# sair-lab/localization

Hardware: AMD Instinct MI355X
Metric: localization updates/sec (8-anchor UWB, batch=65k) (higher is better)
Workload: dtype f64

## Files before the change

### include/localization_amd.h

```cpp
#ifndef LOCALIZATION_AMD_H
#define LOCALIZATION_AMD_H

#include <stddef.h>
#include <stdint.h>

#ifdef __cplusplus
extern "C" {
#endif

#define LOC_ABI_VERSION 4

typedef enum loc_status {
    LOC_OK = 0,
    LOC_ERR_INVALID = -1,
    LOC_ERR_NO_DEVICE = -2,
    LOC_ERR_HIP = -3,
    LOC_ERR_UNKNOWN_NODE = -4,
    LOC_ERR_UNSUPPORTED = -5,
    LOC_ERR_SINGULAR = -6
} loc_status;

enum { LOC_JAC_ANALYTIC = 0, LOC_JAC_NUMERIC_G2O = 1 };

const char* loc_last_error(void);
// ... 33 lines not shown

int loc_snapshot_set_positions(loc_snapshot* s, const double* pos_soa_host);
int loc_snapshot_get_positions(loc_snapshot* s, double* pos_soa_host);
void* loc_snapshot_positions_device(loc_snapshot* s);
int64_t loc_snapshot_epochs_done(const loc_snapshot* s);
int loc_snapshot_set_epochs_done(loc_snapshot* s, int64_t epochs);

int loc_snapshot_pack_ranges_host(const loc_snapshot* s, int32_t epochs, const float* src_kmb, float* dst_tiles,
                                  float pad_value);

int loc_snapshot_solve_device(loc_snapshot* s, int32_t epochs, const float* dist_dev, const float* err_dev,
                              double* out_pos_dev, double* out_chi2_dev, uint8_t* out_trials_dev,
                              void* hip_stream);

int loc_snapshot_solve_host(loc_snapshot* s, int32_t epochs, const float* dist_tiles_host,
                            const float* err_tiles_host, double* out_pos_host, double* out_chi2_host,
                            uint8_t* out_trials_host);

int loc_snapshot_solve_host_kmb(loc_snapshot* s, int32_t epochs, const float* dist_kmb_host, const float* err_kmb_host,
                                double* out_pos_host, double* out_chi2_host, uint8_t* out_trials_host);

int loc_snapshot_solve_device_cov(loc_snapshot* s, int32_t epochs, const float* dist_dev, const float* err_dev,
                                  double* out_pos_dev, double* out_chi2_dev, uint8_t* out_trials_dev,
                                  double* out_cov_dev, int32_t* out_cov_mask_dev, int32_t* out_cov_status_dev, void* hip_stream);
int loc_snapshot_solve_host_kmb_cov(loc_snapshot* s, int32_t epochs, const float* dist_kmb_host, const float* err_kmb_host,
                                    double* out_pos_host, double* out_chi2_host, uint8_t* out_trials_host,
                                    double* out_cov_host, int32_t* out_cov_mask_host, int32_t* out_cov_status_host);

int loc_host_alloc(void** out, size_t bytes);
int loc_host_free(void* p);

int loc_snapshot_timing_begin(loc_snapshot* s, int32_t max_launches);
int loc_snapshot_timing_end(loc_snapshot* s, int32_t* n_launches, double* total_ms, double* avg_ms);


typedef struct loc_window loc_window;
typedef struct loc_window_caps {
    int32_t nv_max, nr_max, np_max, ns_max;
    int32_t bw_max;
} loc_window_caps;

int loc_window_create(loc_window** out, int32_t device, int64_t batch, const loc_window_caps* caps,
                      int32_t n_anchors, const double* anchors_xyz_host, int32_t maximum_iteration);
int loc_window_destroy(loc_window* w);
int loc_window_set_anchors(loc_window* w, int32_t n_anchors, const double* anchors_xyz_host);
size_t loc_window_lds_bytes(const loc_window_caps* caps);
int loc_window_solve_host(loc_window* w, int64_t n_instances, const int32_t* counts, double* poses,
                          const int32_t* r_idx, const double* r_val, const int32_t* p_idx, const double* p_val,
                          const int32_t* s_idx, const double* s_val, double* result);
int loc_window_last_kernel_ms(loc_window* w, double* ms);
int loc_window_set_endpoint1_offsets(loc_window* w, int64_t n_instances, const double* off1_xyz);
int loc_window_set_prior_information(loc_window* w, int64_t n_instances, const double* pinfo);
int loc_window_set_jacobian(loc_window* w, int32_t jacobian);
int loc_window_set_ordering(loc_window* w, int32_t natural);
int loc_window_set_chain_threshold(loc_window* w, int64_t min_batch);
enum { LOC_WINDOW_KERNEL_NONE = -1, LOC_WINDOW_KERNEL_GENERAL = 0, LOC_WINDOW_KERNEL_CHAIN = 1, LOC_WINDOW_KERNEL_CHAIN3 = 2, LOC_WINDOW_KERNEL_ARROW3 = 3, LOC_WINDOW_KERNEL_TREE = 4,
       LOC_WINDOW_KERNEL_TREE_LANE = 5 ,
       LOC_WINDOW_KERNEL_WAVE3 = 6 ,
       LOC_WINDOW_KERNEL_WAVE6 = 7 ,
       LOC_WINDOW_KERNEL_WAVE6S = 8  };
int loc_window_last_kernel_kind(const loc_window* w, int32_t* kind);
int loc_window_set_option(loc_window* w, const char* name, int64_t value);
int loc_window_last_host_timing(const loc_window* w, double* validate_topology_run_cached);
int loc_window_upload(loc_window* w, int64_t n_instances, const int32_t* counts, const double* poses,
                      const int32_t* r_idx, const double* r_val, const int32_t* p_idx, const double* p_val,
                      const int32_t* s_idx, const double* s_val);
// ... 193 lines not shown
```

### localization_amd/_lib.py

```python
import ctypes as C
import os

_HERE = os.path.dirname(os.path.abspath(__file__))
_SO = os.environ.get("LOCALIZATION_AMD_LIB") or os.path.join(_HERE, "liblocalization_amd.so")
_LIB = None

LOC_OK = 0
LOC_ERR_NO_DEVICE = -2
JAC_ANALYTIC = 0
JAC_NUMERIC_G2O = 1


class LocalizationAmdError(RuntimeError):
    def __init__(self, code, msg):
        super().__init__(f"localization_amd error {code}: {msg}")
        self.code = code


class SnapshotParams(C.Structure):
    _fields_ = [("maximum_iteration", C.c_int32), ("distance_outlier", C.c_double), ("gate_warmup_epochs", C.c_int32), ("jacobian", C.c_int32),
                ("lanes_per_instance", C.c_int32), ("block_threads", C.c_int32)]


class FusionParams(C.Structure):
    _fields_ = [("maximum_iteration", C.c_int32), ("distance_outlier", C.c_double), ("gate_warmup_epochs", C.c_int32),
                ("antenna_offset", C.c_double * 3), ("block_threads", C.c_int32), ("jacobian", C.c_int32)]


def library_path():
    return _SO


EXPORTED_SYMBOLS = [
    "loc_last_error", "loc_abi_version", "loc_device_count", "loc_shard_bounds", "loc_shard_plan",
    "loc_snapshot_default_params", "loc_snapshot_create", "loc_snapshot_destroy", "loc_snapshot_batch",
    "loc_snapshot_anchor_groups", "loc_snapshot_lanes_per_instance", "loc_snapshot_range_floats",
    "loc_snapshot_set_positions", "loc_snapshot_get_positions", "loc_snapshot_positions_device",
    "loc_snapshot_epochs_done", "loc_snapshot_set_epochs_done",
    "loc_snapshot_pack_ranges_host", "loc_snapshot_solve_device", "loc_snapshot_solve_host",
    "loc_snapshot_solve_host_kmb", "loc_snapshot_solve_device_cov", "loc_snapshot_solve_host_kmb_cov", "loc_host_alloc", "loc_host_free",
    "loc_snapshot_timing_begin", "loc_snapshot_timing_end",
    "loc_window_create", "loc_window_destroy", "loc_window_set_anchors", "loc_window_lds_bytes", "loc_window_solve_host",
    "loc_window_last_kernel_ms", "loc_window_set_endpoint1_offsets", "loc_window_set_prior_information", "loc_window_set_jacobian", "loc_window_set_ordering", "loc_window_set_chain_threshold", "loc_window_last_kernel_kind", "loc_window_set_option", "loc_window_last_host_timing", "loc_window_upload", "loc_window_upload_dev",
    "loc_window_solve_resident", "loc_window_download", "loc_window_poses_device", "loc_window_result_device",
    "loc_window_timing_begin", "loc_window_timing_end",
    "loc_window_covariance_host", "loc_window_covariance_resident", "loc_window_last_covariance_ms", "loc_window_covariance_plan",
    "loc_window_marginal_prior_host", "loc_window_joint_covariance_host", "loc_window_joint_covariance_resident", "loc_window_joint_covariance_plan",
    "loc_window_slide_resident", "loc_window_slide_resident_dev", "loc_window_slide_plain_resident_dev", "loc_window_download_tables",
    "loc_window_edge_chi2_host", "loc_window_edge_chi2_resident", "loc_window_prune_resident",
    "loc_window_publish_resident", "loc_window_path_resident",
    "loc_window_set_message_config", "loc_window_message_rows_dev", "loc_window_push_messages_resident_dev",
    "loc_node_default_config", "loc_node_create", "loc_node_destroy", "loc_node_add_range", "loc_node_add_imu",
    "loc_node_add_pose", "loc_node_add_twist", "loc_node_add_lidar", "loc_node_add_rl_range", "loc_node_solve", "loc_node_get_path",
    "loc_node_number_measurements", "loc_node_last_timing", "loc_node_last_kernel_kind", "loc_node_flush_tail", "loc_node_set_deferred", "loc_node_solve_pending", "loc_nodes_solve_batch",
    "loc_nodes_release_batch_cache",
    "loc_fusion_default_params", "loc_fusion_create", "loc_fusion_destroy", "loc_fusion_set_poses", "loc_fusion_get_poses",
    "loc_fusion_solve_device", "loc_fusion_solve_host", "loc_fusion_solve_host_kmb", "loc_fusion_last_kernel_ms", "loc_fusion_timing_begin", "loc_fusion_timing_end",
    "loc_fusion_solve_device_cov", "loc_fusion_solve_host_kmb_cov",
]


def lib():
    global _LIB
    if _LIB is not None:
        return _LIB
    if not os.path.exists(_SO):
        raise LocalizationAmdError(-100, f"{_SO} is missing: build it with `python -c 'import __graft_entry__ as g; "
                                   "g.build()'` (hipcc --offload-arch=gfx950). There is no CPU fallback.")
    L = C.CDLL(_SO)
    vp, dp, fp = C.c_void_p, C.POINTER(C.c_double), C.POINTER(C.c_float)
    L.loc_last_error.restype = C.c_char_p
    L.loc_abi_version.restype = C.c_int32
    L.loc_device_count.restype = C.c_int32
    L.loc_shard_bounds.argtypes = [C.c_int64, C.c_int32, C.c_int32, C.POINTER(C.c_int64), C.POINTER(C.c_int64)]
    L.loc_shard_plan.argtypes = [C.c_int64, C.c_int32, C.c_int32, C.c_void_p]
    L.loc_snapshot_default_params.argtypes = [C.POINTER(SnapshotParams)]
    L.loc_snapshot_default_params.restype = None
    L.loc_snapshot_create.argtypes = [C.POINTER(vp), C.c_int32, C.c_int64, C.c_int32, dp, C.POINTER(SnapshotParams)]
    L.loc_snapshot_destroy.argtypes = [vp]
    L.loc_snapshot_batch.argtypes = [vp]; L.loc_snapshot_batch.restype = C.c_int64
    L.loc_snapshot_anchor_groups.argtypes = [vp]; L.loc_snapshot_anchor_groups.restype = C.c_int32
    L.loc_snapshot_lanes_per_instance.argtypes = [vp]; L.loc_snapshot_lanes_per_instance.restype = C.c_int32
    L.loc_snapshot_range_floats.argtypes = [vp, C.c_int32]; L.loc_snapshot_range_floats.restype = C.c_size_t
    L.loc_snapshot_set_positions.argtypes = [vp, dp]
    L.loc_snapshot_get_positions.argtypes = [vp, dp]
    L.loc_snapshot_positions_device.argtypes = [vp]; L.loc_snapshot_positions_device.restype = vp
    L.loc_snapshot_epochs_done.argtypes = [vp]; L.loc_snapshot_epochs_done.restype = C.c_int64
    L.loc_snapshot_set_epochs_done.argtypes = [vp, C.c_int64]
    L.loc_snapshot_pack_ranges_host.argtypes = [vp, C.c_int32, fp, fp, C.c_float]
    L.loc_snapshot_solve_device.argtypes = [vp, C.c_int32, vp, vp, vp, vp, vp, vp]
    L.loc_snapshot_solve_host.argtypes = [vp, C.c_int32, fp, fp, dp, dp, C.POINTER(C.c_uint8)]
    L.loc_snapshot_solve_host_kmb.argtypes = [vp, C.c_int32, vp, vp, vp, vp, vp]
    L.loc_snapshot_solve_device_cov.argtypes = [vp, C.c_int32] + [vp] * 9
    L.loc_snapshot_solve_host_kmb_cov.argtypes = [vp, C.c_int32] + [vp] * 8
    L.loc_host_alloc.argtypes = [C.POINTER(vp), C.c_size_t]
    L.loc_host_free.argtypes = [vp]
    L.loc_snapshot_timing_begin.argtypes = [vp, C.c_int32]
    L.loc_snapshot_timing_end.argtypes = [vp, C.POINTER(C.c_int32), dp, dp]
    ip = C.POINTER(C.c_int32)
    L.loc_window_create.argtypes = [C.POINTER(vp), C.c_int32, C.c_int64, vp, C.c_int32, dp, C.c_int32]
    L.loc_window_destroy.argtypes = [vp]
    L.loc_window_set_anchors.argtypes = [vp, C.c_int32, dp]
    L.loc_window_lds_bytes.argtypes = [vp]; L.loc_window_lds_bytes.restype = C.c_size_t
    L.loc_window_solve_host.argtypes = [vp, C.c_int64, ip, dp, ip, dp, ip, dp, ip, dp, dp]
    L.loc_window_last_kernel_ms.argtypes = [vp, dp]
    L.loc_window_set_jacobian.argtypes = [vp, C.c_int32]
    L.loc_window_set_endpoint1_offsets.argtypes = [vp, C.c_int64, dp]
    L.loc_window_set_prior_information.argtypes = [vp, C.c_int64, dp]
    L.loc_window_set_ordering.argtypes = [vp, C.c_int32]
    L.loc_window_set_chain_threshold.argtypes = [vp, C.c_int64]
    L.loc_window_last_kernel_kind.argtypes = [vp, ip]
    L.loc_window_upload.argtypes = [vp, C.c_int64, ip, dp, ip, dp, ip, dp, ip, dp]
    L.loc_window_upload_dev.argtypes = [vp, vp, C.c_int64] + [vp] * 9
    L.loc_window_solve_resident.argtypes = [vp, vp]
    L.loc_window_download.argtypes = [vp, dp, dp]
    L.loc_window_poses_device.argtypes = [vp]; L.loc_window_poses_device.restype = vp
    L.loc_window_result_device.argtypes = [vp]; L.loc_window_result_device.restype = vp
    L.loc_window_timing_begin.argtypes = [vp, C.c_int32]
    L.loc_window_timing_end.argtypes = [vp, ip, dp, dp]
    L.loc_window_covariance_host.argtypes = [vp, C.c_int64, ip, dp, ip, dp, ip, dp, ip, dp, dp, ip, ip]
    L.loc_window_marginal_prior_host.argtypes = [vp, C.c_int64, ip, dp, ip, dp, ip, dp, ip, dp, ip, ip, dp, dp, dp, ip, ip]
    L.loc_window_covariance_resident.argtypes = [vp, vp, vp, vp, vp]
    L.loc_window_last_covariance_ms.argtypes = [vp, dp]
    L.loc_window_covariance_plan.argtypes = [vp, C.c_int64, ip, ip, ip, C.POINTER(C.c_int64), C.POINTER(C.c_size_t)]
    L.loc_window_joint_covariance_host.argtypes = [vp, C.c_int64, ip, dp, ip, dp, ip, dp, ip, dp, C.c_int32, ip, ip, dp, ip, ip, dp]
    L.loc_window_joint_covariance_resident.argtypes = [vp, vp, C.c_int32, ip, ip, vp, vp, vp, vp]
    L.loc_window_joint_covariance_plan.argtypes = [vp, C.c_int64, ip, ip, ip, C.c_int32, ip, ip, C.POINTER(C.c_int64), C.POINTER(C.c_size_t)]
    L.loc_window_set_option.argtypes = [vp, C.c_char_p, C.c_int64]
    L.loc_window_slide_resident.argtypes = [vp, vp, ip, dp, C.c_int32, ip, ip, dp, C.c_int32, ip, dp, vp, vp, vp, vp]
    L.loc_window_slide_resident_dev.argtypes = [vp, vp, vp, vp, C.c_int32, vp, vp, vp, C.c_int32, vp, vp, vp, vp, vp, vp, vp]
    L.loc_window_slide_plain_resident_dev.argtypes = [vp, vp, vp, vp, C.c_int32, vp, vp, vp, C.c_int32, vp, vp, C.c_int32, vp, vp, vp, vp, vp]
# ... 134 lines not shown
```

### localization_amd/csrc/capi.cpp

```cpp
#include <algorithm>
#include <cmath>
#include <cstdio>
#include <cstring>
#include <new>
#include <string>
#include <vector>

#include "capi_host.h"
#include "snapshot_kernel.h"

static thread_local std::string g_last_error;

int locamd_fail(int code, const char* what) {
    g_last_error = what ? what : "";
    return code;
}
int locamd_fail_hip(hipError_t e, const char* where) {
    g_last_error = std::string(where) + ": " + hipGetErrorString(e);
    return LOC_ERR_HIP;
}

struct loc_snapshot {
    int device = 0;
    long long B = 0;
    int M = 0, M4 = 0, M_PAD = 0;
    int lpi = 1;
    loc_snapshot_params prm{};
    double* d_anchors = nullptr;
    double* d_pos = nullptr;
    hipStream_t own_stream = nullptr;
    float *d_dist = nullptr, *d_err = nullptr;
    double *d_out_pos = nullptr, *d_out_chi2 = nullptr;
    uint8_t* d_out_trials = nullptr;
    size_t staged_epochs = 0;
    long long epochs_done = 0;
    locamd::HostPipeline pipe;
    locamd::LaunchTimer timer;
};

extern "C" {

const char* loc_last_error(void) { return g_last_error.c_str(); }
int32_t loc_abi_version(void) { return LOC_ABI_VERSION; }

int32_t loc_device_count(void) {
    int n = 0;
    if (hipGetDeviceCount(&n) != hipSuccess) return 0;
    return n;
}

int loc_shard_bounds(int64_t total, int32_t rank, int32_t world, int64_t* lo, int64_t* hi) {
    if (total < 0 || world <= 0 || rank < 0 || rank >= world || !lo || !hi) return locamd_fail(LOC_ERR_INVALID, "loc_shard_bounds arguments");
    const int64_t per = (total + world - 1) / world;
    const int64_t a = rank * per < total ? rank * per : total;
    *lo = a;
    *hi = a + per < total ? a + per : total;
    return LOC_OK;
}

int loc_shard_plan(int64_t total, int32_t world, int32_t devices_per_node, loc_shard* out) {
    if (total < 0 || world <= 0 || !out) return locamd_fail(LOC_ERR_INVALID, "loc_shard_plan arguments");
    if (devices_per_node <= 0) {
        devices_per_node = loc_device_count();
        if (devices_per_node <= 0) return locamd_fail(LOC_ERR_NO_DEVICE, "no HIP device visible: pass devices_per_node explicitly");
    }
    for (int32_t r = 0; r < world; ++r) {
        out[r].rank = r; out[r].world = world; out[r].device = r % devices_per_node; out[r].reserved = 0;
        const int rc = loc_shard_bounds(total, r, world, &out[r].lo, &out[r].hi);
// ... 105 lines not shown
    if (!s || !src || !dst || epochs <= 0) return locamd_fail(LOC_ERR_INVALID, "pack_ranges");
    const size_t B = (size_t)s->B;
    for (int k = 0; k < epochs; ++k)
        for (int g = 0; g < s->M4; ++g)
            for (int j = 0; j < 4; ++j) {
                const int m = 4 * g + j;
                float* d = dst + (((size_t)k * s->M4 + g) * B) * 4 + j;
                if (m < s->M) {
                    const float* sp = src + ((size_t)k * s->M + m) * B;
                    for (size_t b = 0; b < B; ++b) d[4 * b] = sp[b];
                } else {
                    for (size_t b = 0; b < B; ++b) d[4 * b] = pad_value;
                }
            }
    return LOC_OK;
}

}

static int solve_device(loc_snapshot* s, int32_t epochs, const float* dist_dev, const float* err_dev, double* out_pos_dev,
                        double* out_chi2_dev, uint8_t* out_trials_dev, double* cov, int32_t* cov_mask, int32_t* cov_status, void* hip_stream) {
    if (epochs <= 0 || !dist_dev || !err_dev || !out_pos_dev || !out_chi2_dev) return locamd_fail(LOC_ERR_INVALID, "solve arguments");
    if (((uintptr_t)dist_dev | (uintptr_t)err_dev) & 15u) return locamd_fail(LOC_ERR_INVALID, "range tiles must be 16-byte aligned");
    LOC_HIP(hipSetDevice(s->device));
    hipStream_t st = hip_stream ? (hipStream_t)hip_stream : s->own_stream;
    locamd::SnapshotArgs a;
    a.dist = dist_dev; a.err = err_dev; a.pos = s->d_pos; a.out_pos = out_pos_dev; a.out_chi2 = out_chi2_dev;
    a.out_trials = out_trials_dev; a.anchors = s->d_anchors; a.B = s->B; a.K = epochs; a.M4 = s->M4;
    a.iterations = s->prm.maximum_iteration; a.gate = s->prm.distance_outlier;
    {
        long long left = (long long)s->prm.gate_warmup_epochs - s->epochs_done;
        a.gate_from_epoch = left > 0 ? (int)(left > epochs ? epochs : left) : 0;
    }
    LOC_HIP(s->timer.start(st));
    hipError_t e;
    if (!cov) {
        e = locamd::launch_snapshot(a, s->M_PAD, s->lpi, s->prm.jacobian, s->prm.block_threads, st);
    } else {
        locamd::SnapshotCovArgs ca;
        static_cast<locamd::SnapshotArgs&>(ca) = a;
        ca.out_cov = cov; ca.out_cov_mask = cov_mask; ca.out_cov_status = cov_status;
        e = locamd::launch_snapshot_cov(ca, s->M_PAD, s->lpi, s->prm.jacobian, s->prm.block_threads, st);
    }
    if (e != hipSuccess) return locamd_fail_hip(e, "launch_snapshot");
    LOC_HIP(s->timer.stop(st));
    s->epochs_done += epochs;
    return LOC_OK;
}

extern "C" {

int loc_snapshot_solve_device(loc_snapshot* s, int32_t epochs, const float* dist_dev, const float* err_dev,
                              double* out_pos_dev, double* out_chi2_dev, uint8_t* out_trials_dev, void* hip_stream) {
    if (!s) return locamd_fail(LOC_ERR_INVALID, "null handle");
    return solve_device(s, epochs, dist_dev, err_dev, out_pos_dev, out_chi2_dev, out_trials_dev, nullptr, nullptr, nullptr, hip_stream);
}

int loc_snapshot_solve_device_cov(loc_snapshot* s, int32_t epochs, const float* dist_dev, const float* err_dev,
                                  double* out_pos_dev, double* out_chi2_dev, uint8_t* out_trials_dev,
                                  double* out_cov_dev, int32_t* out_cov_mask_dev, int32_t* out_cov_status_dev, void* hip_stream) {
    if (!s) return locamd_fail(LOC_ERR_INVALID, "null handle");
    if (!out_cov_dev || !out_cov_mask_dev || !out_cov_status_dev) return locamd_fail(LOC_ERR_INVALID, "covariance outputs: all three are required");
    return solve_device(s, epochs, dist_dev, err_dev, out_pos_dev, out_chi2_dev, out_trials_dev, out_cov_dev, out_cov_mask_dev,
                        out_cov_status_dev, hip_stream);
}

// ... 38 lines not shown
                     return solve_device(s, kc, s->d_dist + toff, s->d_err + toff, s->d_out_pos + 3 * o, s->d_out_chi2 + o, s->d_out_trials + o,
                                         cov_h ? p.d_cov + 6 * o : nullptr, cov_h ? p.d_cov_mask + o : nullptr, cov_h ? p.d_cov_status + o : nullptr, s->own_stream);
                 });
}

extern "C" {

int loc_snapshot_solve_host_kmb(loc_snapshot* s, int32_t epochs, const float* dist_kmb, const float* err_kmb,
                                double* out_pos_h, double* out_chi2_h, uint8_t* out_trials_h) {
    if (!s) return locamd_fail(LOC_ERR_INVALID, "null handle");
    return solve_host_kmb(s, epochs, dist_kmb, err_kmb, out_pos_h, out_chi2_h, out_trials_h, nullptr, nullptr, nullptr);
}

int loc_snapshot_solve_host_kmb_cov(loc_snapshot* s, int32_t epochs, const float* dist_kmb, const float* err_kmb,
                                    double* out_pos_h, double* out_chi2_h, uint8_t* out_trials_h,
                                    double* out_cov_h, int32_t* out_cov_mask_h, int32_t* out_cov_status_h) {
    if (!s) return locamd_fail(LOC_ERR_INVALID, "null handle");
    if (!out_cov_h || !out_cov_mask_h || !out_cov_status_h) return locamd_fail(LOC_ERR_INVALID, "covariance outputs: all three are required");
    return solve_host_kmb(s, epochs, dist_kmb, err_kmb, out_pos_h, out_chi2_h, out_trials_h, out_cov_h, out_cov_mask_h, out_cov_status_h);
}

int loc_host_alloc(void** out, size_t bytes) {
    if (!out || bytes == 0) return locamd_fail(LOC_ERR_INVALID, "loc_host_alloc");
    *out = nullptr;
    LOC_HIP(hipHostMalloc(out, bytes, hipHostMallocDefault));
    return LOC_OK;
}
int loc_host_free(void* p) {
    if (!p) return LOC_OK;
    LOC_HIP(hipHostFree(p));
    return LOC_OK;
}

int loc_snapshot_timing_begin(loc_snapshot* s, int32_t max_launches) {
    return s ? s->timer.begin(s->device, max_launches) : locamd_fail(LOC_ERR_INVALID, "timing_begin");
}
int loc_snapshot_timing_end(loc_snapshot* s, int32_t* n_launches, double* total_ms, double* avg_ms) {
    return s ? s->timer.end(s->device, n_launches, total_ms, avg_ms) : locamd_fail(LOC_ERR_INVALID, "timing_end");
}

}
```

### localization_amd/csrc/lm_damping.h

```cpp
#pragma once
#include <hip/hip_runtime.h>
#include <math.h>

namespace locamd {
namespace {

constexpr double lm_tau = 1e-5;
constexpr double lm_good_lo = 1.0 / 3.0;
constexpr double lm_good_hi = 2.0 / 3.0;
constexpr int lm_max_trials = 10;
constexpr double lm_scale_eps = 1e-3;

__device__ __forceinline__ double lm_lambda_accepted(double lambda, double rho) {
    const double r21 = 2.0 * rho - 1.0;
    double alpha = 1.0 - r21 * r21 * r21;
    alpha = fmin(alpha, lm_good_hi);
    return lambda * fmax(lm_good_lo, alpha);
}

}
}
```

### localization_amd/csrc/snapshot_kernel.h

```cpp
#pragma once
#include <hip/hip_runtime.h>
#include <stdint.h>

namespace locamd {

struct SnapshotArgs {
    const float* dist;
    const float* err;
    double* pos;
    double* out_pos;
    double* out_chi2;
    uint8_t* out_trials;
    const double* anchors;
    long long B;
    int K;
    int M4;
    int iterations;
    double gate;
    int gate_from_epoch;
};

struct SnapshotCovArgs : SnapshotArgs {
    double* out_cov;
    int32_t* out_cov_mask;
    int32_t* out_cov_status;
};

hipError_t launch_snapshot(const SnapshotArgs& a, int m_pad, int lpi, int jac, int block_threads, hipStream_t stream);
hipError_t launch_snapshot_cov(const SnapshotCovArgs& a, int m_pad, int lpi, int jac, int block_threads, hipStream_t stream);
bool snapshot_supported(int m_pad, int lpi);
hipError_t launch_pack_kmb(const float* src_kmb, float* dst_tiles, long long B, int M, int M4, int K, float pad, hipStream_t stream);

}
```

### localization_amd/csrc/snapshot_kernel.hip

```cpp
#include "snapshot_kernel.h"
#include "device_math.h"
#include "lm_damping.h"
#include "cov_device.h"

#include <float.h>
#include <math.h>

#include <type_traits>

namespace locamd {

namespace {

template <int CTRL>
__device__ __forceinline__ double dpp_move(double v) {
    int lo = __double2loint(v), hi = __double2hiint(v);
    lo = __builtin_amdgcn_update_dpp(0, lo, CTRL, 0xF, 0xF, false);
    hi = __builtin_amdgcn_update_dpp(0, hi, CTRL, 0xF, 0xF, false);
    return __hiloint2double(hi, lo);
}
constexpr int DPP_QUAD_XOR1 = 0xB1;
constexpr int DPP_QUAD_XOR2 = 0x4E;
constexpr int DPP_ROW_HALF_MIRROR = 0x141;

template <int LPI>
__device__ __forceinline__ double group_sum(double v) {
    if constexpr (LPI >= 2) v += dpp_move<DPP_QUAD_XOR1>(v);
    if constexpr (LPI >= 4) v += dpp_move<DPP_QUAD_XOR2>(v);
    if constexpr (LPI >= 8) v += dpp_move<DPP_ROW_HALF_MIRROR>(v);
    return v;
}
template <int LPI>
__device__ __forceinline__ double group_prod(double v) {
    if constexpr (LPI >= 2) v *= dpp_move<DPP_QUAD_XOR1>(v);
    if constexpr (LPI >= 4) v *= dpp_move<DPP_QUAD_XOR2>(v);
    if constexpr (LPI >= 8) v *= dpp_move<DPP_ROW_HALF_MIRROR>(v);
    return v;
}

struct System {
    double h00, h01, h02, h11, h12, h22;
    double b0, b1, b2;
    double rchi;
    double chi;
};

#pragma clang fp contract(off)
__device__ __forceinline__ double range_norm_plain(double dx, double dy, double dz) {
    return sqrt_ieee_unscaled(dx * dx + dy * dy + dz * dz);
}
__device__ __forceinline__ double range_sq_plain(double dx, double dy, double dz) { return dx * dx + dy * dy + dz * dz; }
#pragma clang fp contract(fast)

template <int LPI, int APL, int JAC>
__device__ __forceinline__ System evaluate(const double px, const double py, const double pz,
                                           const double (&ax)[APL], const double (&ay)[APL], const double (&az)[APL],
                                           const double (&d)[APL], double (&w)[APL], const double gate) {
    System s = {0, 0, 0, 0, 0, 0, 0, 0, 0, 0, 0};
    double prod = 1.0;
    int kexp = 0;
#pragma unroll
    for (int j = 0; j < APL; ++j) {
        const double dx = px - ax[j], dy = py - ay[j], dz = pz - az[j];
        double n, jx, jy, jz;
        if constexpr (JAC == 0) {
            const double n2 = fmax(dx * dx + dy * dy + dz * dz, 1e-300);
            double inv;
            sqrt_and_rsqrt_fast(n2, n, inv);
            jx = -dx * inv; jy = -dy * inv; jz = -dz * inv;
        } else {
// ... 72 lines not shown
    if constexpr (APL % 4 == 0) {
#pragma unroll
        for (int q4 = 0; q4 < APL / 4; ++q4) {
            const long long idx = (k * a.M4 + (m0 / 4 + q4)) * B + inst;
            const float4 dv = reinterpret_cast<const float4*>(a.dist)[idx];
            const float4 sv = reinterpret_cast<const float4*>(a.err)[idx];
            df[4 * q4 + 0] = dv.x; df[4 * q4 + 1] = dv.y; df[4 * q4 + 2] = dv.z; df[4 * q4 + 3] = dv.w;
            sf[4 * q4 + 0] = sv.x; sf[4 * q4 + 1] = sv.y; sf[4 * q4 + 2] = sv.z; sf[4 * q4 + 3] = sv.w;
        }
    } else if constexpr (APL == 2) {
        const long long idx = ((k * a.M4 + m0 / 4) * B + inst) * 2 + (m0 % 4) / 2;
        const float2 dv = reinterpret_cast<const float2*>(a.dist)[idx];
        const float2 sv = reinterpret_cast<const float2*>(a.err)[idx];
        df[0] = dv.x; df[1] = dv.y; sf[0] = sv.x; sf[1] = sv.y;
    } else {
        static_assert(APL == 1 || APL == 2 || APL % 4 == 0, "anchors per lane");
        const long long idx = ((k * a.M4 + m0 / 4) * B + inst) * 4 + (m0 % 4);
        df[0] = a.dist[idx]; sf[0] = a.err[idx];
    }
}
template <int APL>
__device__ __forceinline__ void ingest(const float (&df)[APL], const float (&sf)[APL], double (&d)[APL], double (&w)[APL]) {
#pragma unroll
    for (int j = 0; j < APL; ++j) {
        const double dd = (double)df[j], ss = (double)sf[j];
        const bool valid = (ss > 0.0) && (ss < DBL_MAX) && (fabs(dd) < DBL_MAX);
        const double cov = valid ? ss * ss : 1.0;
        const double mask = valid ? 1.0 : 0.0;
        d[j] = valid ? dd : 0.0;
        w[j] = fast_rcp(cov) * mask;
    }
}

template <int APL> struct SnapshotLds {
    static constexpr int NEXT_BYTES = APL * 256 * 16;
    static constexpr int RAW_BYTES = (APL % 4 == 0) ? (2 * (APL / 4) * 256 * 16) : 0;
    static constexpr int BYTES = NEXT_BYTES + RAW_BYTES;
};

typedef __attribute__((address_space(3))) void* lds_void_ptr;
typedef const __attribute__((address_space(1))) void* glb_void_ptr;

template <int LPI, int APL, int JAC, bool COV>
__global__ void __launch_bounds__(256) snapshot_lm_kernel(const std::conditional_t<COV, SnapshotCovArgs, SnapshotArgs> a) {
    __shared__ __attribute__((aligned(16))) char lds_bytes[SnapshotLds<APL>::BYTES];
    double2* const s_next = reinterpret_cast<double2*>(lds_bytes);
    float4* const s_raw = reinterpret_cast<float4*>(lds_bytes + SnapshotLds<APL>::NEXT_BYTES);
    const int tib = threadIdx.x;
    const long long tid = (long long)blockIdx.x * blockDim.x + tib;
    const long long inst = tid / LPI;
    const int g = (int)(tid % LPI);
    const long long B = a.B;
    const int K = a.K;
    const bool live = (inst < B) && K > 0;
    const long long ld_inst = live ? inst : 0;
    bool exhausted = !live;

    double ax[APL], ay[APL], az[APL];
    const int m0 = g * APL;
#pragma unroll
    for (int j = 0; j < APL; ++j) {
        ax[j] = a.anchors[(m0 + j) * 3 + 0];
        ay[j] = a.anchors[(m0 + j) * 3 + 1];
        az[j] = a.anchors[(m0 + j) * 3 + 2];
    }

    auto put_next = [&](const double (&dd)[APL], const double (&ww)[APL]) {
#pragma unroll
        for (int j = 0; j < APL; ++j) s_next[j * 256 + tib] = make_double2(dd[j], ww[j]);
    };
    auto take_next = [&](double (&dd)[APL], double (&ww)[APL]) {
        typedef double v2f64 __attribute__((ext_vector_type(2)));
        const unsigned addr = (unsigned)(unsigned long long)(s_next + tib);
        v2f64 v[APL];
#pragma unroll
        for (int j = 0; j < APL; ++j) asm volatile("ds_read_b128 %0, %1 offset:%2" : "=v"(v[j]) : "v"(addr), "n"(j * 4096));
        if constexpr (APL == 8) {
            asm volatile("s_waitcnt lgkmcnt(0)" : "+v"(v[0]), "+v"(v[1]), "+v"(v[2]), "+v"(v[3]), "+v"(v[4]), "+v"(v[5]), "+v"(v[6]), "+v"(v[7]) :: "memory");
        } else {
#pragma unroll
// ... 28 lines not shown
            }
        } else {
            load_epoch<APL>(a, ke, m0, ld_inst, df, sf);
        }
        ingest<APL>(df, sf, dd, ww);
    };

    double px = 0, py = 0, pz = 0;
    double d[APL], w[APL];
    if (live) { px = a.pos[0 * B + inst]; py = a.pos[1 * B + inst]; pz = a.pos[2 * B + inst]; }
    {
        float df0[APL], sf0[APL];
        load_epoch<APL>(a, 0, m0, ld_inst, df0, sf0);
        ingest<APL>(df0, sf0, d, w);
        if (K > 1) {
            double dn[APL], wn[APL];
            load_epoch<APL>(a, 1, m0, ld_inst, df0, sf0);
            ingest<APL>(df0, sf0, dn, wn);
            put_next(dn, wn);
        }
        if (K > 2) prefetch(2);
    }
    asm volatile("" : "+v"(px), "+v"(py), "+v"(pz));

    System cur = {1, 0, 0, 1, 0, 1, 0, 0, 0, 0, 0};
    double cur_chi = 0, last_chi = 0, lambda = 1.0, ni = 2.0;
    int c = 0;
    int k = 0;
    int it = 0, q = 0, trials = 0;
    bool init = true;
    bool waiting = false;

    while (__any(!exhausted)) {
        const bool active = !exhausted && !waiting;
        double x0, x1, x2;
        const bool ok2 = solve3(cur, lambda, x0, x1, x2) && !init;
        if (!ok2) { x0 = 0.0; x1 = 0.0; x2 = 0.0; }
        const double tx = px + x0, ty = py + x1, tz = pz + x2;
        const bool gate_now = active && init && (a.gate > 0.0) && (k >= a.gate_from_epoch);
        const System tr = evaluate<LPI, APL, JAC>(tx, ty, tz, ax, ay, az, d, w, gate_now ? a.gate : DBL_MAX);

        const bool first = active && init;
        const bool lm = active && !init;
        const double temp_chi = ok2 ? tr.rchi : DBL_MAX;
        double scale = x0 * __builtin_fma(lambda, x0, cur.b0) + x1 * __builtin_fma(lambda, x1, cur.b1) +
                       x2 * __builtin_fma(lambda, x2, cur.b2);
        scale += lm_scale_eps;
        const double rho = (cur_chi - temp_chi) * fast_rcp(scale);
        const bool accept = lm && (rho > 0.0) && (fabs(temp_chi) < DBL_MAX) && ok2;
        if (first || accept) {
            cur = tr;
            cur_chi = tr.rchi;
            px = tx; py = ty; pz = tz;
        }
        const double lam_acc = lm_lambda_accepted(lambda, rho);
        const double lam_first = lm_tau * fmax(fabs(tr.h00), fmax(fabs(tr.h11), fabs(tr.h22)));
        lambda = first ? lam_first : (accept ? lam_acc : (lm ? lambda * ni : lambda));
        ni = (first || accept) ? 2.0 : (lm ? ni * 2.0 : ni);
        last_chi = active ? tr.chi : last_chi;
        trials = first ? 0 : trials + (lm ? 1 : 0);
        q = first ? 0 : q + (lm ? 1 : 0);
        const bool end_iter = lm && !((rho < 0.0) && (q < lm_max_trials));
        it = first ? 0 : it + (end_iter ? 1 : 0);
        const bool finished = (first && ((a.iterations <= 0) || !((tr.h00 + tr.h11 + tr.h22) > 0.0))) ||
                              (end_iter && ((q == lm_max_trials) || (rho == 0.0) || (it >= a.iterations)));
        q = end_iter ? 0 : q;
        init = active ? false : init;

        if (__any(finished)) {
            if (finished) {
                if (g == 0) {
                    a.out_pos[((long long)k * 3 + 0) * B + inst] = px;
                    a.out_pos[((long long)k * 3 + 1) * B + inst] = py;
                    a.out_pos[((long long)k * 3 + 2) * B + inst] = pz;
                    a.out_chi2[(long long)k * B + inst] = last_chi;
                    if (a.out_trials) a.out_trials[(long long)k * B + inst] = (uint8_t)(trials > 255 ? 255 : trials);
                    if constexpr (COV) {
                        double hc[6] = {cur.h00, cur.h01, cur.h02, cur.h11, cur.h12, cur.h22};
                        int msk;
                        const bool cok = cov_invert_packed<3>(hc, msk);
#pragma unroll
                        for (int i = 0; i < 6; ++i) a.out_cov[((long long)k * 6 + i) * B + inst] = hc[i];
                        a.out_cov_mask[(long long)k * B + inst] = msk;
                        a.out_cov_status[(long long)k * B + inst] = cok ? 0 : -6;
                    }
                }
                if (k + 1 >= K) {
                    exhausted = true;
                    if (g == 0) { a.pos[0 * B + inst] = px; a.pos[1 * B + inst] = py; a.pos[2 * B + inst] = pz; }
                } else if (k == c) {
                    take_next(d, w);
                    k = c + 1;
                    init = true;
                } else {
                    waiting = true;
                }
            }
        }
        if (!__any(!exhausted && k == c)) {
            ++c;
            if (c + 1 < K) {
                double dn[APL], wn[APL];
                consume(c + 1, dn, wn);
                put_next(dn, wn);
                asm volatile("" ::: "memory");
                if (c + 2 < K) prefetch(c + 2);
                if (waiting) {
#pragma unroll
                    for (int j = 0; j < APL; ++j) { d[j] = dn[j]; w[j] = wn[j]; }
                    k = c + 1;
                    init = true;
                    waiting = false;
                }
            }
        }
    }
}

template <int LPI, int APL, int JAC, bool COV, class Args>
hipError_t launch_one(const Args& a, int block_threads, hipStream_t stream) {
    const long long lanes = a.B * LPI;
    const long long blocks = (lanes + block_threads - 1) / block_threads;
    if (blocks <= 0 || blocks > 0x7fffffffLL) return hipErrorInvalidValue;
    hipLaunchKernelGGL((snapshot_lm_kernel<LPI, APL, JAC, COV>), dim3((unsigned)blocks), dim3((unsigned)block_threads), 0, stream, a);
    return hipGetLastError();
}

template <int LPI, int APL, bool COV, class Args>
hipError_t launch_jac(const Args& a, int jac, int block_threads, hipStream_t stream) {
    return jac == 0 ? launch_one<LPI, APL, 0, COV>(a, block_threads, stream) : launch_one<LPI, APL, 1, COV>(a, block_threads, stream);
}

template <bool COV, class Args>
hipError_t launch_mapping(const Args& a, int m_pad, int lpi, int jac, int block_threads, hipStream_t stream) {
    if (!snapshot_supported(m_pad, lpi)) return hipErrorInvalidValue;
    if (block_threads <= 0) block_threads = 256;
    if (block_threads % 64 || block_threads > 256) return hipErrorInvalidValue;
    switch (m_pad * 100 + lpi) {
        case 401: return launch_jac<1, 4, COV>(a, jac, block_threads, stream);
        case 402: return launch_jac<2, 2, COV>(a, jac, block_threads, stream);
        case 404: return launch_jac<4, 1, COV>(a, jac, block_threads, stream);
        case 801: return launch_jac<1, 8, COV>(a, jac, block_threads, stream);
        case 802: return launch_jac<2, 4, COV>(a, jac, block_threads, stream);
        case 804: return launch_jac<4, 2, COV>(a, jac, block_threads, stream);
        case 808: return launch_jac<8, 1, COV>(a, jac, block_threads, stream);
        case 1201: return launch_jac<1, 12, COV>(a, jac, block_threads, stream);
// ... 58 lines not shown
```

### localization_amd/snapshot.py

```python
import ctypes as C

import numpy as np

from . import _lib
from ._lib import SnapshotParams, check, lib


def pack_ranges(x_kmb, pad_value=0.0):
    x = np.ascontiguousarray(x_kmb, dtype=np.float32)
    K, M, B = x.shape
    M4 = (M + 3) // 4
    out = np.full((K, M4 * 4, B), pad_value, dtype=np.float32)
    out[:, :M, :] = x
    return np.ascontiguousarray(out.reshape(K, M4, 4, B).transpose(0, 1, 3, 2))


def unpack_ranges(tiles, M):
    t = np.asarray(tiles)
    K, M4, B, _ = t.shape
    return np.ascontiguousarray(t.transpose(0, 1, 3, 2).reshape(K, M4 * 4, B)[:, :M, :])


class SnapshotSolver(_lib.EpochSolver):
    _prefix = "loc_snapshot"

    def __init__(self, anchors, batch, maximum_iteration=10, distance_outlier=1.0, jacobian="numeric",
                 lanes_per_instance=0, block_threads=0, device=0, gate_warmup_epochs=1):
        import torch
        self.torch = torch
        L = lib()
        if L.loc_device_count() <= 0 or not torch.cuda.is_available():
            raise _lib.LocalizationAmdError(_lib.LOC_ERR_NO_DEVICE,
                                            "no HIP device visible: localization_amd has no CPU fallback")
        anchors = np.ascontiguousarray(anchors, dtype=np.float64)
        assert anchors.ndim == 2 and anchors.shape[1] == 3
        self.M = anchors.shape[0]
        self.B = int(batch)
        self.device = int(device)
        self.dev = torch.device("cuda", self.device)
        prm = SnapshotParams()
        L.loc_snapshot_default_params(C.byref(prm))
        prm.maximum_iteration = int(maximum_iteration)
        prm.distance_outlier = float(distance_outlier)
        prm.gate_warmup_epochs = int(gate_warmup_epochs)
        prm.jacobian = {"analytic": _lib.JAC_ANALYTIC, "numeric": _lib.JAC_NUMERIC_G2O,
                        "numeric_g2o": _lib.JAC_NUMERIC_G2O}[jacobian]
        prm.lanes_per_instance = int(lanes_per_instance)
        prm.block_threads = int(block_threads)
        h = C.c_void_p()
        check(L.loc_snapshot_create(C.byref(h), self.device, self.B, self.M,
                                    anchors.ctypes.data_as(C.POINTER(C.c_double)), C.byref(prm)))
        self.h = h
        self.L = L
        self.M4 = L.loc_snapshot_anchor_groups(h)
        self.lanes_per_instance = L.loc_snapshot_lanes_per_instance(h)

    def set_positions(self, pos_3b):
        p = np.ascontiguousarray(pos_3b, dtype=np.float64)
        assert p.shape == (3, self.B)
        check(self.L.loc_snapshot_set_positions(self.h, p.ctypes.data_as(C.POINTER(C.c_double))))

    def get_positions(self):
        p = np.zeros((3, self.B), dtype=np.float64)
        check(self.L.loc_snapshot_get_positions(self.h, p.ctypes.data_as(C.POINTER(C.c_double))))
        return p

    def to_device_tiles(self, x_kmb, pad_value=0.0):
        return self.torch.from_numpy(pack_ranges(x_kmb, pad_value)).to(self.dev)

    def alloc_outputs(self, K, trials=True, covariance=False):
        return self._device_outputs(K, 3, 6, trials, covariance)

    def solve_device(self, dist_tiles, err_tiles, out_pos, out_chi2, out_trials=None, out_cov=None, out_cov_mask=None, out_cov_status=None):
        t = self.torch
        K = dist_tiles.shape[0]
        assert tuple(dist_tiles.shape) == (K, self.M4, self.B, 4) and dist_tiles.dtype == t.float32
        assert tuple(err_tiles.shape) == tuple(dist_tiles.shape) and err_tiles.dtype == t.float32
        assert dist_tiles.is_contiguous() and err_tiles.is_contiguous()
        assert tuple(out_pos.shape) == (K, 3, self.B) and out_pos.dtype == t.float64 and out_pos.is_contiguous()
        assert tuple(out_chi2.shape) == (K, self.B) and out_chi2.dtype == t.float64 and out_chi2.is_contiguous()
        if out_trials is not None:
            assert tuple(out_trials.shape) == (K, self.B) and out_trials.dtype == t.uint8
        for x in (dist_tiles, err_tiles, out_pos, out_chi2):
            assert x.device == self.dev
        cov = self._cov_device_args((out_cov, out_cov_mask, out_cov_status), K, 6, self.dev)
        fn = self.L.loc_snapshot_solve_device_cov if cov else self.L.loc_snapshot_solve_device
        check(fn(self.h, K, dist_tiles.data_ptr(), err_tiles.data_ptr(), out_pos.data_ptr(), out_chi2.data_ptr(),
                 out_trials.data_ptr() if out_trials is not None else None, *cov, C.c_void_p(t.cuda.current_stream(self.dev).cuda_stream)))
# ... 27 lines not shown
```

Measured before the change: 1.996 billion.

## Let idle wavefront lanes speculatively run LM damping trials for stalled lanes

When some lanes in a wavefront are exhausted or waiting while another lane is stuck retrying rejected Levenberg-Marquardt steps, the idle lanes borrow that lane's linear system and try successive lambda values from the rejection ladder in parallel. The first helper whose trial ends the iteration has its state copied back to the owner via readlane, which shortens the serial trial chain that causes divergence in the wave. The cost is a large amount of cross-lane traffic each loop, extra LDS to save the helpers' own positions, and added register pressure. Optional per-wave counters record how often helping happens.

Result: slower. 1.900 billion (-4.8%).

```diff
diff --git a/include/localization_amd.h b/include/localization_amd.h
--- a/include/localization_amd.h
+++ b/include/localization_amd.h
@@ -89,6 +89,10 @@
 
 int loc_snapshot_timing_begin(loc_snapshot* s, int32_t max_launches);
 int loc_snapshot_timing_end(loc_snapshot* s, int32_t* n_launches, double* total_ms, double* avg_ms);
+
+int loc_snapshot_set_option(loc_snapshot* s, const char* name, int64_t value);
+int64_t loc_snapshot_counter_words(const loc_snapshot* s);
+int loc_snapshot_set_counters(loc_snapshot* s, uint32_t* counters_dev, int64_t words);
 
 
 typedef struct loc_window loc_window;
diff --git a/localization_amd/_lib.py b/localization_amd/_lib.py
--- a/localization_amd/_lib.py
+++ b/localization_amd/_lib.py
@@ -40,6 +40,7 @@
     "loc_snapshot_pack_ranges_host", "loc_snapshot_solve_device", "loc_snapshot_solve_host",
     "loc_snapshot_solve_host_kmb", "loc_snapshot_solve_device_cov", "loc_snapshot_solve_host_kmb_cov", "loc_host_alloc", "loc_host_free",
     "loc_snapshot_timing_begin", "loc_snapshot_timing_end",
+    "loc_snapshot_set_option", "loc_snapshot_counter_words", "loc_snapshot_set_counters",
     "loc_window_create", "loc_window_destroy", "loc_window_set_anchors", "loc_window_lds_bytes", "loc_window_solve_host",
     "loc_window_last_kernel_ms", "loc_window_set_endpoint1_offsets", "loc_window_set_prior_information", "loc_window_set_jacobian", "loc_window_set_ordering", "loc_window_set_chain_threshold", "loc_window_last_kernel_kind", "loc_window_set_option", "loc_window_last_host_timing", "loc_window_upload", "loc_window_upload_dev",
     "loc_window_solve_resident", "loc_window_download", "loc_window_poses_device", "loc_window_result_device",
@@ -97,6 +98,9 @@
     L.loc_host_free.argtypes = [vp]
     L.loc_snapshot_timing_begin.argtypes = [vp, C.c_int32]
     L.loc_snapshot_timing_end.argtypes = [vp, C.POINTER(C.c_int32), dp, dp]
+    L.loc_snapshot_set_option.argtypes = [vp, C.c_char_p, C.c_int64]
+    L.loc_snapshot_counter_words.argtypes = [vp]; L.loc_snapshot_counter_words.restype = C.c_int64
+    L.loc_snapshot_set_counters.argtypes = [vp, vp, C.c_int64]
     ip = C.POINTER(C.c_int32)
     L.loc_window_create.argtypes = [C.POINTER(vp), C.c_int32, C.c_int64, vp, C.c_int32, dp, C.c_int32]
     L.loc_window_destroy.argtypes = [vp]
diff --git a/localization_amd/csrc/capi.cpp b/localization_amd/csrc/capi.cpp
--- a/localization_amd/csrc/capi.cpp
+++ b/localization_amd/csrc/capi.cpp
@@ -34,6 +34,8 @@
     uint8_t* d_out_trials = nullptr;
     size_t staged_epochs = 0;
     long long epochs_done = 0;
+    int trial_helpers = 1;
+    uint32_t* d_counters = nullptr;
     locamd::HostPipeline pipe;
     locamd::LaunchTimer timer;
 };
@@ -205,6 +207,7 @@
         long long left = (long long)s->prm.gate_warmup_epochs - s->epochs_done;
         a.gate_from_epoch = left > 0 ? (int)(left > epochs ? epochs : left) : 0;
     }
+    a.trial_helpers = s->trial_helpers; a.counters = s->d_counters;
     LOC_HIP(s->timer.start(st));
     hipError_t e;
     if (!cov) {
@@ -309,6 +312,22 @@
     return LOC_OK;
 }
 
+int loc_snapshot_set_option(loc_snapshot* s, const char* name, int64_t value) {
+    if (!s || !name) return locamd_fail(LOC_ERR_INVALID, "loc_snapshot_set_option arguments");
+    if (!std::strcmp(name, "trial_helpers")) { s->trial_helpers = value != 0; return LOC_OK; }
+    return locamd_fail(LOC_ERR_INVALID, "loc_snapshot_set_option: unknown option");
+}
+int64_t loc_snapshot_counter_words(const loc_snapshot* s) {
+    return s ? locamd::kSnapshotCounterWords * locamd::snapshot_waves(s->B, s->lpi, s->prm.block_threads) : 0;
+}
+int loc_snapshot_set_counters(loc_snapshot* s, uint32_t* counters_dev, int64_t words) {
+    if (!s) return locamd_fail(LOC_ERR_INVALID, "null handle");
+    if (counters_dev && (words < loc_snapshot_counter_words(s) || ((uintptr_t)counters_dev & 3u)))
+        return locamd_fail(LOC_ERR_INVALID, "loc_snapshot_set_counters: block smaller than loc_snapshot_counter_words, or misaligned");
+    s->d_counters = counters_dev;
+    return LOC_OK;
+}
+
 int loc_snapshot_timing_begin(loc_snapshot* s, int32_t max_launches) {
     return s ? s->timer.begin(s->device, max_launches) : locamd_fail(LOC_ERR_INVALID, "timing_begin");
 }
diff --git a/localization_amd/csrc/lm_damping.h b/localization_amd/csrc/lm_damping.h
--- a/localization_amd/csrc/lm_damping.h
+++ b/localization_amd/csrc/lm_damping.h
@@ -1,6 +1,12 @@
 #pragma once
 #include <hip/hip_runtime.h>
 #include <math.h>
+
+#if defined(__HIPCC__)
+#define LOCAMD_LM_HD __host__ __device__
+#else
+#define LOCAMD_LM_HD
+#endif
 
 namespace locamd {
 namespace {
@@ -18,5 +24,29 @@
     return lambda * fmax(lm_good_lo, alpha);
 }
 
+
+LOCAMD_LM_HD inline void lm_reject_step(double& lambda, double& nu) {
+    lambda *= nu;
+    nu *= 2.0;
+}
+LOCAMD_LM_HD inline void lm_reject_ladder(double& lambda, double& nu, int steps) {
+    for (int i = 0; i < lm_max_trials - 1; ++i) {
+        double l = lambda, n = nu;
+        lm_reject_step(l, n);
+        lambda = i < steps ? l : lambda;
+        nu = i < steps ? n : nu;
+    }
+}
+LOCAMD_LM_HD inline bool lm_trial_ends(double rho, int q) { return !((rho < 0.0) && (q < lm_max_trials)); }
+LOCAMD_LM_HD inline int lm_ladder_helpers(int q, int idle) {
+    const int room = lm_max_trials - 1 - q;
+    return idle < room ? (idle < 0 ? 0 : idle) : (room < 0 ? 0 : room);
+}
+LOCAMD_LM_HD inline int lm_ladder_winner(bool own_ends, unsigned long long helper_ends, unsigned long long helpers) {
+    if (own_ends || helpers == 0) return -1;
+    helper_ends &= helpers;
+    return helper_ends ? __builtin_ctzll(helper_ends) : 63 - __builtin_clzll(helpers);
+}
+
 }
 }
diff --git a/localization_amd/csrc/snapshot_kernel.h b/localization_amd/csrc/snapshot_kernel.h
--- a/localization_amd/csrc/snapshot_kernel.h
+++ b/localization_amd/csrc/snapshot_kernel.h
@@ -18,7 +18,15 @@
     int iterations;
     double gate;
     int gate_from_epoch;
+    int trial_helpers;
+    uint32_t* counters;
 };
+constexpr int kSnapshotCounterWords = 4;
+constexpr bool snapshot_trial_helpers(int lpi, int apl) { return lpi == 1 && apl <= 8; }
+inline long long snapshot_waves(long long B, int lpi, int block_threads) {
+    const long long lanes = B * lpi, blocks = (lanes + block_threads - 1) / block_threads;
+    return blocks * (block_threads / 64);
+}
 
 struct SnapshotCovArgs : SnapshotArgs {
     double* out_cov;
diff --git a/localization_amd/csrc/snapshot_kernel.hip b/localization_amd/csrc/snapshot_kernel.hip
--- a/localization_amd/csrc/snapshot_kernel.hip
+++ b/localization_amd/csrc/snapshot_kernel.hip
@@ -36,6 +36,12 @@
     if constexpr (LPI >= 4) v *= dpp_move<DPP_QUAD_XOR2>(v);
     if constexpr (LPI >= 8) v *= dpp_move<DPP_ROW_HALF_MIRROR>(v);
     return v;
+}
+
+__device__ __forceinline__ int lane_value(int v, int lane) { return __builtin_amdgcn_readlane(v, lane); }
+__device__ __forceinline__ double lane_value(double v, int lane) {
+    const int lo = __builtin_amdgcn_readlane(__double2loint(v), lane), hi = __builtin_amdgcn_readlane(__double2hiint(v), lane);
+    return __hiloint2double(hi, lo);
 }
 
 struct System {
@@ -174,10 +180,11 @@
     }
 }
 
-template <int APL> struct SnapshotLds {
+template <int APL, int LPI> struct SnapshotLds {
     static constexpr int NEXT_BYTES = APL * 256 * 16;
     static constexpr int RAW_BYTES = (APL % 4 == 0) ? (2 * (APL / 4) * 256 * 16) : 0;
-    static constexpr int BYTES = NEXT_BYTES + RAW_BYTES;
+    static constexpr int OWN_BYTES = snapshot_trial_helpers(LPI, APL) ? 3 * 256 * 8 : 0;
+    static constexpr int BYTES = NEXT_BYTES + RAW_BYTES + OWN_BYTES;
 };
 
 typedef __attribute__((address_space(3))) void* lds_void_ptr;
@@ -185,9 +192,12 @@
 
 template <int LPI, int APL, int JAC, bool COV>
 __global__ void __launch_bounds__(256) snapshot_lm_kernel(const std::conditional_t<COV, SnapshotCovArgs, SnapshotArgs> a) {
-    __shared__ __attribute__((aligned(16))) char lds_bytes[SnapshotLds<APL>::BYTES];
+    typedef SnapshotLds<APL, LPI> Lds;
+    constexpr bool HELPERS = snapshot_trial_helpers(LPI, APL);
+    __shared__ __attribute__((aligned(16))) char lds_bytes[Lds::BYTES];
     double2* const s_next = reinterpret_cast<double2*>(lds_bytes);
-    float4* const s_raw = reinterpret_cast<float4*>(lds_bytes + SnapshotLds<APL>::NEXT_BYTES);
+    float4* const s_raw = reinterpret_cast<float4*>(lds_bytes + Lds::NEXT_BYTES);
+    [[maybe_unused]] double* const s_own = reinterpret_cast<double*>(lds_bytes + Lds::NEXT_BYTES + Lds::RAW_BYTES);
     const int tib = threadIdx.x;
     const long long tid = (long long)blockIdx.x * blockDim.x + tib;
     const long long inst = tid / LPI;
@@ -282,7 +292,42 @@
     bool waiting = false;
 
     while (__any(!exhausted)) {
-        const bool active = !exhausted && !waiting;
+        bool helping = false;
+        int help_lane = -1;
+        if constexpr (HELPERS) {
+            if (a.trial_helpers) {
+                const unsigned long long stalled = __ballot(!exhausted && !waiting && !init && q >= 1);
+                const unsigned long long idle = __ballot(exhausted || waiting);
+                if (stalled != 0 && idle != 0) {
+                    const int h = __builtin_ctzll(stalled);
+                    const int q_h = lane_value(q, h);
+                    const int n = lm_ladder_helpers(q_h, __popcll(idle));
+                    if (n > 0) {
+                        help_lane = h;
+                        const int rank = __builtin_amdgcn_mbcnt_hi((unsigned)(idle >> 32), __builtin_amdgcn_mbcnt_lo((unsigned)idle, 0));
+                        helping = (exhausted || waiting) && rank < n;
+                        const int j = helping ? rank + 1 : 0;
+                        if (helping) { s_own[tib] = px; s_own[256 + tib] = py; s_own[512 + tib] = pz; }
+                        auto lend = [&](double& v) { const double hv = lane_value(v, h); v = helping ? hv : v; };
+                        lend(cur.h00); lend(cur.h01); lend(cur.h02); lend(cur.h11); lend(cur.h12); lend(cur.h22);
+                        lend(cur.b0); lend(cur.b1); lend(cur.b2); lend(cur.rchi); lend(cur.chi);
+                        lend(cur_chi); lend(px); lend(py); lend(pz);
+#pragma unroll
+                        for (int i = 0; i < APL; ++i) { lend(d[i]); lend(w[i]); }
+                        double lam = lane_value(lambda, h), nu = lane_value(ni, h);
+                        lm_reject_ladder(lam, nu, j);
+                        lambda = helping ? lam : lambda;
+                        ni = helping ? nu : ni;
+                        const int it_h = lane_value(it, h), trials_h = lane_value(trials, h);
+                        q = helping ? q_h + j : q;
+                        it = helping ? it_h : it;
+                        trials = helping ? trials_h + j : trials;
+                        init = helping ? false : init;
+                    }
+                }
+            }
+        }
+        const bool active = (!exhausted && !waiting) || helping;
         double x0, x1, x2;
         const bool ok2 = solve3(cur, lambda, x0, x1, x2) && !init;
         if (!ok2) { x0 = 0.0; x1 = 0.0; x2 = 0.0; }
@@ -310,12 +355,40 @@
         last_chi = active ? tr.chi : last_chi;
         trials = first ? 0 : trials + (lm ? 1 : 0);
         q = first ? 0 : q + (lm ? 1 : 0);
-        const bool end_iter = lm && !((rho < 0.0) && (q < lm_max_trials));
+        const bool end_iter = lm && lm_trial_ends(rho, q);
         it = first ? 0 : it + (end_iter ? 1 : 0);
-        const bool finished = (first && ((a.iterations <= 0) || !((tr.h00 + tr.h11 + tr.h22) > 0.0))) ||
-                              (end_iter && ((q == lm_max_trials) || (rho == 0.0) || (it >= a.iterations)));
+        bool finished = (first && ((a.iterations <= 0) || !((tr.h00 + tr.h11 + tr.h22) > 0.0))) ||
+                        (end_iter && ((q == lm_max_trials) || (rho == 0.0) || (it >= a.iterations)));
         q = end_iter ? 0 : q;
         init = active ? false : init;
+
+        [[maybe_unused]] int adopted = 0;
+        if constexpr (HELPERS) {
+            if (help_lane >= 0) {
+                const int lane = tib & 63;
+                const unsigned long long helpers = __ballot(helping);
+                const unsigned long long ends = __ballot(end_iter || !(fabs(tr.chi) < DBL_MAX));
+                const int win = lm_ladder_winner((ends >> help_lane) & 1, ends, helpers);
+                if (win >= 0) {
+                    const bool me = lane == help_lane;
+                    adopted = __popcll(helpers & ((2ull << win) - 1));
+                    const bool win_finished = (__ballot(finished) >> win) & 1;
+                    auto take = [&](double& v) { const double wv = lane_value(v, win); v = me ? wv : v; };
+                    auto take_int = [&](int& v) { const int wv = lane_value(v, win); v = me ? wv : v; };
+                    take(cur.h00); take(cur.h01); take(cur.h02); take(cur.h11); take(cur.h12); take(cur.h22);
+                    take(cur.b0); take(cur.b1); take(cur.b2); take(cur.rchi); take(cur.chi);
+                    take(cur_chi); take(px); take(py); take(pz); take(lambda); take(ni); take(last_chi);
+#pragma unroll
+                    for (int i = 0; i < APL; ++i) take(w[i]);
+                    take_int(q); take_int(it); take_int(trials);
+                    finished = me ? win_finished : finished;
+                }
+                if (helping) {
+                    px = s_own[tib]; py = s_own[256 + tib]; pz = s_own[512 + tib];
+                    finished = false;
+                }
+            }
+        }
 
         if (__any(finished)) {
             if (finished) {
@@ -362,6 +435,13 @@
                     init = true;
                     waiting = false;
                 }
+            }
+        }
+        if constexpr (HELPERS) {
+            if (a.counters && (tib & 63) == 0) {
+                uint32_t* const cw = a.counters + ((long long)blockIdx.x * (blockDim.x / 64) + tib / 64) * kSnapshotCounterWords;
+                atomicAdd(cw + 0, 1u);
+                if (help_lane >= 0) { atomicAdd(cw + 1, 1u); atomicAdd(cw + 2, (uint32_t)adopted); }
             }
         }
     }
diff --git a/localization_amd/snapshot.py b/localization_amd/snapshot.py
--- a/localization_amd/snapshot.py
+++ b/localization_amd/snapshot.py
@@ -25,7 +25,7 @@
     _prefix = "loc_snapshot"
 
     def __init__(self, anchors, batch, maximum_iteration=10, distance_outlier=1.0, jacobian="numeric",
-                 lanes_per_instance=0, block_threads=0, device=0, gate_warmup_epochs=1):
+                 lanes_per_instance=0, block_threads=0, device=0, gate_warmup_epochs=1, trial_helpers=True):
         import torch
         self.torch = torch
         L = lib()
@@ -54,6 +54,18 @@
         self.L = L
         self.M4 = L.loc_snapshot_anchor_groups(h)
         self.lanes_per_instance = L.loc_snapshot_lanes_per_instance(h)
+        self._counters = None
+        if not trial_helpers:
+            self.set_option("trial_helpers", 0)
+
+    def set_option(self, name, value):
+        check(self.L.loc_snapshot_set_option(self.h, str(name).encode(), int(value)))
+
+    def enable_counters(self, on=True):
+        t = self.torch
+        self._counters = t.zeros((self.L.loc_snapshot_counter_words(self.h) // 4, 4), dtype=t.int32, device=self.dev) if on else None
+        check(self.L.loc_snapshot_set_counters(self.h, self._counters.data_ptr() if on else None, self._counters.numel() if on else 0))
+        return self._counters
 
     def set_positions(self, pos_3b):
         p = np.ascontiguousarray(pos_3b, dtype=np.float64)
```
